# Bricktricker/gpu-solve

Measured on AMD Instinct MI355X. Metric: MLUPS (Jacobi smoother) + V-cycle wall-time, 512³ fp64; achieved HBM GB/s %peak, higher is better.
Workload: dtype f64

## Files before the change

### gpu-solve_amd/csrc/gs_capi.cpp

```cpp
#include <algorithm>
#include <array>
#include <chrono>
#include <cstdlib>
#include <cmath>
#include <cstring>
#include <iostream>
#include <memory>
#include <string>
#include <thread>
#include <vector>

#include <hip/hip_runtime.h>

#include "gpusolve_driver.h"
#include "gs_grid.hpp"

namespace {

thread_local std::string g_err;

template <class F>
int guarded(F&& f)
{
    try {
// ... 136 lines not shown
        if (residual) *residual = r;
    });
}

int gs_grid_jacobi(void* grid, int level, int sweeps)
{
    return guarded([&] { gs::HipSolver::jacobi(G(grid), (std::size_t)level, (std::size_t)sweeps); });
}

int gs_grid_residual_norm(void* grid, int level, double* norm)
{
    return guarded([&] {
        const double r = gs::HipSolver::compResidual(G(grid), (std::size_t)level, false, true);
        if (norm) *norm = r;
    });
}

int gs_grid_num_levels(void* grid) { return (int)G(grid).numLevels(); }

int gs_grid_level_fused(void* grid, int level)
{
    if (level < 0 || level >= (int)G(grid).numLevels()) return 0;
    return G(grid).getLevel(level).fusedPairs ? 1 : 0;
}

int gs_grid_level(void* grid, int level, gs_level* out)
{
    if (level < 0 || level >= (int)G(grid).numLevels() || !out) return 1;
    *out = G(grid).getLevel(level).geom;
    return 0;
}

static double* field_ptr(void* grid, int level, int field, bool writable)
{
    auto& g = G(grid);
    if (level < 0 || level >= (int)g.numLevels()) return nullptr;
    auto& L = g.getLevel(level);
    switch (field) {
    case 0: return L.v ? L.v.data() : nullptr;
    case 1: return L.restV ? L.restV.data() : nullptr;
    case 2:
        if (writable) g.newtonVTouched();
        return L.newtonV ? L.newtonV.data() : nullptr;
    case 3: return L.f ? L.f.data() : nullptr;
    case 4: return L.r ? L.r.data() : nullptr;
    case 5: return (level == 0 && g.newtonF) ? g.newtonF.data() : nullptr;
// ... 388 lines not shown
```

### gpu-solve_amd/csrc/gs_device.hpp

```cpp
#pragma once
#include <hip/hip_runtime.h>
#include <math.h>

#include <cmath>
#include <stdint.h>
#include <stdlib.h>

#include <map>
#include <mutex>
#include <utility>

#include "gpusolve_hip.h"

#ifdef GS_EXP_NOEXP
#define exp(x) ((x) * 1.0000001)
#endif
#ifdef GS_EXP_NOBAR
#define GS_LDS_BARRIER() __builtin_amdgcn_s_waitcnt(0xc07f)
#else
#define GS_LDS_BARRIER()                                                                                               \
    do {                                                                                                               \
        __builtin_amdgcn_s_waitcnt(0xc07f);                                                                            \
        __builtin_amdgcn_s_barrier();                                                                                  \
    } while (0)
// ... 118 lines not shown
{
    const unsigned e = ((unsigned)__double2hiint(s) >> 20) & 0x7ffu;
    if (k.fastdiv && e - 124u < 1500u) {
        const double y = hh_recip(k.hh);
        const double q = s * y;
        const double r = __builtin_fma(-k.hh, q, s);
        return __builtin_fma(r, y, q);
    }
    return s / k.hh;
}

__device__ __forceinline__ bool div_hh_fast_ok(double s)
{
    const unsigned e = ((unsigned)__double2hiint(s) >> 20) & 0x7ffu;
    return e - 124u < 1500u;
}
template <int N>
__device__ __forceinline__ void div_hh_n(const Coef& k, double (&s)[N])
{
    bool ok = k.fastdiv;
#pragma unroll
    for (int i = 0; i < N; i++) ok &= div_hh_fast_ok(s[i]);
    if (ok) {
        const double y = hh_recip(k.hh);
#pragma unroll
        for (int i = 0; i < N; i++) {
            const double q = s[i] * y;
            const double r = __builtin_fma(-k.hh, q, s[i]);
            s[i] = __builtin_fma(r, y, q);
        }
    } else {
#pragma unroll
        for (int i = 0; i < N; i++) s[i] = s[i] / k.hh;
    }
}

template <int MODE>
__device__ __forceinline__ void div_hh_row(const Coef& k, double (&q)[2])
{
    if (MODE == GS_NEWTON) {
        q[0] = div_hh(k, q[0]);
        q[1] = div_hh(k, q[1]);
    } else {
        div_hh_n(k, q);
    }
}
// ... 2329 lines not shown
        if (lane == 0) red[wid] = sumsq;
        __syncthreads();
        if (tid == 0) {
            double t = 0.0;
            for (int i = 0; i < 2 * WX; i++) t += red[i];
            partials[tile] = t;
        }
    }
    if constexpr (TS) {
        if (tid == 0) {
            double* t = const_cast<double*>(es) + 4 * tile;
            t[0] = (double)tstart;
            t[1] = (double)wall_clock64();
            t[2] = (double)(blockIdx.x + (int64_t)gridDim.x * blockIdx.y);
            t[3] = (double)(unsigned)__builtin_amdgcn_s_getreg((31 << 11) | 4);
        }
    }
}

constexpr int TBY_RY = 2, TBY_RY_NEWTON = 2, TBY_WX = 4, TB_RY_B = 2, TB_WX_B = 8;
constexpr int tby_pfd(int mode) { return mode == GS_LINEAR ? 2 : 1; }
bool tbx_pfd2() { return kKnobs.tbxPfd2; }

bool xh_enabled() { return kKnobs.pairXh; }

int64_t resident_blocks(const void* fn, int threads)
{
    static std::mutex m;
    static std::map<std::pair<const void*, int>, int64_t> cache;
    std::lock_guard<std::mutex> lk(m);
    const auto key = std::make_pair(fn, threads);
    auto it = cache.find(key);
    if (it != cache.end()) return it->second;
    int per = 0, dev = 0, cus = 0;
    if (hipOccupancyMaxActiveBlocksPerMultiprocessor(&per, fn, threads, 0) != hipSuccess || per < 1) per = 1;
    if (hipGetDevice(&dev) != hipSuccess ||
        hipDeviceGetAttribute(&cus, hipDeviceAttributeMultiprocessorCount, dev) != hipSuccess || cus < 1)
        cus = 256;
    (void)hipGetLastError();
    return cache[key] = (int64_t)per * cus;
}

int fit_chunk(int64_t tiles, int64_t planes, int64_t cap, int lo, int hi, bool even, double halo)
{
    if (!kKnobs.fitRounds || tiles < 1 || planes < 1 || cap < 1) return 0;
    double best = -1.0;
// ... 178 lines not shown
```

### gpu-solve_amd/csrc/gs_grid.cpp

```cpp
#include "gs_grid.hpp"

#include <algorithm>
#include <chrono>
#include <cmath>
#include <cstdio>
#include <cstdlib>
#include <iostream>
#include <string>
#include <utility>

#include <hip/hip_runtime.h>

#include "gpusolve_driver.h"

namespace gs {

void check(int code, const char* what)
{
    if (code != 0) throw Error(std::string(what) + ": " + gs_strerror(code));
}

DeviceField::DeviceField(int64_t nx, int64_t ny, int64_t nz, hipStream_t s, bool dry) : dry_(dry)
{
    int64_t origin = 0;
// ... 142 lines not shown
    const int nlev = (int)std::floor(std::log((double)mn) / std::log(2.0)) + 1;
    levels_.resize(nlev);
    for (int i = 0; i < 7; i++) {
        stencilAbi.s[i] = stencil.values[i];
        stencilAbi.ox[i] = stencil.getXOffset(i);
        stencilAbi.oy[i] = stencil.getYOffset(i);
        stencilAbi.oz[i] = stencil.getZOffset(i);
    }
    {
        auto on = [](const char* name) { return std::getenv(name) != nullptr; };
        sw.fusedSweeps = !on("GS_NO_FUSED_SWEEPS");
        sw.speculation = !on("GS_NO_SPECULATION");
        sw.fusedProlong = !on("GS_NO_FUSED_PROLONG");
        sw.fusedRR = !on("GS_NO_FUSED_RR");
        sw.zeroGuess = !on("GS_NO_ZERO_GUESS");
        sw.pipeline = !on("GS_NO_PIPELINE");
        sw.newtonFusedUpdate = !on("GS_NO_NEWTON_FUSED_UPDATE");
        sw.newtonB = !on("GS_NO_NEWTON_B");
        if (const char* e = std::getenv("GS_NEWTON_B_FUSED")) sw.newtonBFused = std::atoi(e) != 0;
        sw.newtonG = !on("GS_NO_NEWTON_G");
        if (const char* e = std::getenv("GS_NEWTON_PRO_POINTS")) sw.newtonProPoints = std::strtoll(e, nullptr, 10);
        if (const char* e = std::getenv("GS_TILE_POINTS")) sw.tilePoints = std::strtoll(e, nullptr, 10);
        if (const char* e = std::getenv("GS_HALO_ORDER")) sw.haloOrder = std::atoi(e);
    }
    std::vector<int64_t> nzs, pts;
    for (int l = 0; l < nlev; l++) {
        LevelData& L = levels_[l];
        L.levelDim = l == 0 ? gridDim
                            : std::array<std::size_t, 3>{levels_[l - 1].levelDim[0] / 2, levels_[l - 1].levelDim[1] / 2,
                                                         levels_[l - 1].levelDim[2] / 2};
        nzs.push_back((int64_t)L.levelDim[2]);
        pts.push_back((int64_t)(L.levelDim[0] * L.levelDim[1] * L.levelDim[2]));
    }
    if (agglomeratePoints < 0) {
        const char* e = std::getenv("GS_ZSLAB_MIN_POINTS");
        agglomeratePoints = e ? std::atoll(e) : 32768;
    }
    const SlabPlan plan = planZSlabs(nzs, pts, nranks(), agglomeratePoints);

    const hipStream_t s = stream_.s;
    int64_t maxParts = 1;
    for (int l = 0; l < nlev; l++) {
        LevelData& L = levels_[l];
        const int64_t nx = (int64_t)L.levelDim[0], ny = (int64_t)L.levelDim[1];
        L.distributed = plan.distributed[l];
        L.ranksLo = plan.lo[l];
// ... 5 lines not shown
            L.lo = 1;
            L.hi = (int64_t)L.levelDim[2];
        }
        const int64_t nz = L.hi - L.lo + 1;
        L.h = 1.0 / (L.levelDim[1] + 1);
        L.v = DeviceField(nx, ny, nz, s, dry);
        L.vAlt = DeviceField(nx, ny, nz, s, dry);
        L.f = DeviceField(nx, ny, nz, s, dry);
        if (l + 1 < nlev) L.r = DeviceField(nx, ny, nz, s, dry);
        if (mode == NONLINEAR && l > 0) L.restV = DeviceField(nx, ny, nz, s, dry);
        if (mode == NEWTON) L.newtonV = DeviceField(nx, ny, nz, s, dry);
        if (mode == NEWTON && sw.newtonB && dry) L.bfac = DeviceField(nx, ny, nz, s, dry);
        if (mode == NEWTON && l == 1 && nlev >= 3 && !L.distributed) L.newtonVNext = DeviceField(nx, ny, nz, s, dry);
        L.geom = gs_level{nx, ny, nz, L.v.ldy(), L.v.ldz(), L.lo - 1, L.h};
        maxParts = std::max(maxParts, gs_residual_num_partials(&stencilAbi, &L.geom));
        maxParts = std::max(maxParts, gs_jacobi_sweep2_num_partials(&stencilAbi, &L.geom, (int)mode));
        L.minPlanes = nz;
        if (L.distributed)
            for (int q = 0; q < nranks(); q++) L.minPlanes = std::min(L.minPlanes, L.ranksHi[q] - L.ranksLo[q] + 1);
        gs_level thin = L.geom;
        thin.nz = L.minPlanes;
        L.fusedPairs = sw.fusedSweeps && gs_jacobi_sweep2_supported_mode(&stencilAbi, &thin, (int)mode) == 2 &&
                       (!L.distributed || L.minPlanes >= 2);
        L.tiled = !L.distributed && pts[l] <= sw.tilePoints &&
                  gs_tiled_supported(&stencilAbi, &L.geom, (int)mode) != 0;
    }
    coarseFrom = levels_.size();
    {
        const char* e = std::getenv("GS_COARSE_POINTS");
        const int64_t thr = e ? std::atoll(e) : 512;
        if (thr > 0 && preSmoothing + postSmoothing < (1u << 20))
            for (int l = nlev - 1; l >= 1; l--) {
                if (levels_[l].distributed || pts[l] > thr || nlev - l > gs_coarse_cycle_max_levels()) break;
                coarseFrom = (std::size_t)l;
            }
    }
    if (mode == NEWTON) newtonF = DeviceField(levels_[0].geom.nx, levels_[0].geom.ny, levels_[0].geom.nz, s, dry);
    newtonVZero_ = mode == NEWTON;
    {
        const char* e = std::getenv("GS_METRICS");
        clock.on = !dry && e && *e && *e != '0';
        clock.levelMs.assign(nlev, 0.0);
    }
    if (dry) {
        dryParts_.assign(16, 0.0);
        partials_ = dryParts_.data();
// ... 213 lines not shown
int64_t pairPlanes(HipGridData& g, HipGridData::LevelData& L, int64_t z1, int64_t z2, hipStream_t s,
                   double* partials = nullptr)
{
    if (z2 < z1) return 0;
    gs_level sub = L.geom;
    sub.nz = z2 - z1 + 1;
    sub.z0 += z1 - 1;
    const int64_t off = (z1 - 1) * L.geom.ldz;
    const bool dist = L.distributed && g.nranks() > 1;
    const int zlo = z1 > 1 || (dist && g.rank() > 0);
    const int zhi = z2 < L.geom.nz || (dist && g.rank() + 1 < g.nranks());
    if (g.trace) {
        g.rec("pair", {{"L", (long long)g.levelIndex(L)}, {"z1", z1}, {"z2", z2}, {"zlo", zlo}, {"zhi", zhi},
                       {"vzero", L.vZero}, {"norm", partials != nullptr}});
        return partials ? 1 : 0;
    }
    check(gs_jacobi_sweep2_norm(&g.stencilAbi, &sub, g.kmode(), g.omega, g.gamma, L.vZero ? nullptr : L.v.data() + off,
                                L.vAlt.data() + off, L.f.data() + off, g.wOf(L) ? g.wOf(L) + off : nullptr,
                                zlo, zhi, partials, s),
          "gs_jacobi_sweep2");
    return partials ? gs_jacobi_sweep2_num_partials(&g.stencilAbi, &sub, (int)g.mode) : 0;
}

void proPlanes(HipGridData& g, HipGridData::LevelData& F, HipGridData::LevelData& C, int64_t z1, int64_t z2,
               hipStream_t s)
{
    if (z2 < z1) return;
    gs_level sub = F.geom;
    sub.nz = z2 - z1 + 1;
    sub.z0 += z1 - 1;
    const int64_t off = (z1 - 1) * F.geom.ldz;
    const bool dist = F.distributed && g.nranks() > 1;
    const int zlo = z1 > 1 || (dist && g.rank() > 0);
    const int zhi = z2 < F.geom.nz || (dist && g.rank() + 1 < g.nranks());
    if (g.trace) {
        g.rec("pro", {{"L", (long long)g.levelIndex(F)}, {"z1", z1}, {"z2", z2}, {"zlo", zlo}, {"zhi", zhi}});
        return;
    }
    const int64_t wsn = gs_jacobi_sweep2_prolong_ws_elems(&g.stencilAbi, &sub, (int)g.mode);
    DeviceBuf& wb = F.proWs[s == g.stream() ? 0 : 1];
    if (wsn > wb.size()) throw Error("gs_jacobi_sweep2_prolong: workspace not sized at grid creation");
    double* ws = wsn > 0 ? wb.get(wsn) : nullptr;
    check(gs_jacobi_sweep2_prolong_ws(&g.stencilAbi, &sub, g.kmode(), g.omega, g.gamma, F.v.data() + off,
                                      C.v.data(), nullptr, &C.geom, F.vAlt.data() + off, F.f.data() + off,
                                      g.wOf(F) ? g.wOf(F) + off : nullptr, zlo, zhi, ws, wsn, s),
          "gs_jacobi_sweep2_prolong");
// ... 167 lines not shown
        if ((F.ranksLo[q] - 1) % 2 != 0) return false;
        if (C.distributed && 2 * (C.ranksLo[q] - 1) != F.ranksLo[q] - 1) return false;
    }
    return !C.distributed || grid.vDepth(C) == 2;
}

static bool proWorthIt(HipGridData& grid, std::size_t l)
{
    if (grid.mode != GridParams::NEWTON) return true;
    const int64_t minPoints = grid.sw.newtonProPoints;
    const auto& F = grid.getLevel(l);
    return (int64_t)F.levelDim[0] * (int64_t)F.levelDim[1] * F.minPlanes >= minPoints;
}

void HipSolver::jacobi(HipGridData& grid, std::size_t l, std::size_t sweeps)
{
    auto& L = grid.getLevel(l);
    const hipStream_t s = grid.stream();
    const bool dist = L.distributed && grid.nranks() > 1;
    const int64_t nz = L.geom.nz;
    const int depth = grid.vDepth(L);
    int step = 0;
    while (sweeps > 0) {
        const bool pair = L.fusedPairs && sweeps >= 2;
        const int64_t b = pair ? 2 : depth;
        auto run = [&](int64_t z1, int64_t z2, hipStream_t st) {
            if (pair) pairPlanes(grid, L, z1, z2, st);
            else sweepPlanes(grid, L, z1, z2, st);
        };
        if (!dist) {
            run(1, nz, s);
        } else if (grid.overlapHalo && nz >= 2 * b + 1) {
            hipStream_t bs = s;
            const bool interiorFirst = step > 0 && !grid.haloReady();
            if (!grid.trace) {
                bs = grid.bndStream_.s;
                check((int)hipEventRecord(grid.evA_, s), "hipEventRecord");
            }
            auto interior = [&] {
                if (!grid.trace && step > 0)
                    check((int)hipStreamWaitEvent(s, grid.evBnd_[(step - 1) & 1], 0), "hipStreamWaitEvent");
                run(b + 1, nz - b, s);
            };
            if (interiorFirst) interior();
            if (step > 0) settleExchange(grid);
            if (!grid.trace) {
// ... 532 lines not shown
```

### gpu-solve_amd/csrc/gs_grid.hpp

```cpp
#pragma once
#include <array>
#include <cstddef>
#include <cstdint>
#include <initializer_list>
#include <memory>
#include <string>
#include <functional>
#include <vector>

#include "gpusolve_hip.h"
#include "gs_comm.hpp"
#include "gs_params.hpp"

namespace gs {

void check(int code, const char* what);

class DeviceField {
public:
    DeviceField() = default;
    DeviceField(int64_t nx, int64_t ny, int64_t nz, hipStream_t s, bool dry = false);
    ~DeviceField();
    DeviceField(const DeviceField&) = delete;
    DeviceField& operator=(const DeviceField&) = delete;
// ... 43 lines not shown
    std::vector<hipEvent_t> ev;
    std::vector<int> segLevel;
    void mark(hipStream_t s, int level, bool begin);
    void collect();
    ~LevelClock();
};

class HipGridData final : public GridParams {
public:
    struct LevelData {
        DeviceField v;
        DeviceField vAlt;
        DeviceField restV;
        DeviceField newtonV;
        DeviceField newtonVNext;
        DeviceField f;
        DeviceField r;
        DeviceField bfac;
        std::array<std::size_t, 3> levelDim{};
        double h = 0.0;
        gs_level geom{};
        bool distributed = false;
        bool fusedPairs = false;
        bool vZero = false;
        bool tiled = false;
        int64_t lo = 1, hi = 0;
        int64_t minPlanes = 0;
        std::vector<int64_t> ranksLo, ranksHi;
        std::unique_ptr<DeviceBuf[]> proWs = std::make_unique<DeviceBuf[]>(2);
    };

    explicit HipGridData(const GridParams& grid, Comm* comm = nullptr, int64_t agglomeratePoints = -1,
                         std::vector<std::string>* trace = nullptr);
    ~HipGridData();

    LevelData& getLevel(std::size_t l) { return levels_[l]; }
    const LevelData& getLevel(std::size_t l) const { return levels_[l]; }
    std::size_t numLevels() const { return levels_.size(); }

    DeviceField newtonF;
    gs_stencil stencilAbi{};
    hipStream_t stream() const { return stream_.s; }
    hipStream_t commStream() const { return commStream_.s; }
    Comm* comm() const { return comm_; }
    int rank() const { return comm_ ? comm_->rank() : 0; }
    int nranks() const { return comm_ ? comm_->size() : 1; }
    bool overlapHalo = true;
    struct Switches {
        bool fusedSweeps = true;
        bool speculation = true;
        bool fusedProlong = true;
        bool fusedRR = true;
        bool zeroGuess = true;
        bool pipeline = true;
        bool newtonFusedUpdate = true;
        bool newtonB = true;
        bool newtonBFused = true;
        bool newtonG = true;
        int64_t tilePoints = (int64_t)1 << 18;
        int64_t newtonProPoints = (int64_t)1 << 21;
        int haloOrder = 0;
    } sw;
    std::size_t coarseFrom = 0;
    LevelClock clock;
    std::vector<std::string>* trace = nullptr;
    void rec(const char* op, std::initializer_list<std::pair<const char*, long long>> kv, const char* field = nullptr);
    std::size_t levelIndex(const LevelData& L) const { return (std::size_t)(&L - levels_.data()); }
    static const char* fieldName(const LevelData& L, const DeviceField& f);

    double* partials() const { return partials_; }
    double* dNorm() const { return dNorm_; }
    double* hNormDev() const { return hNormDev_; }
    double* dRankSums() const { return dRankSums_; }
    double readNorm();
    void readNormBegin();
    double readNormEnd();
    void sync();

    int kmode() const { return newtonB_ ? (bconst_ ? (int)GS_NEWTON_G : (int)GS_NEWTON_B) : (int)mode; }
    const double* wOf(const LevelData& L) const
    {
        return newtonB_ ? L.bfac.data() : (L.newtonV ? L.newtonV.data() : nullptr);
    }
// ... 90 lines not shown
```

### gpu-solve_amd/csrc/gs_kernels.hip

```cpp
#include "gs_device.hpp"

extern "C" {

int gs_field_layout(int64_t nx, int64_t ny, int64_t nz, int64_t* ldy, int64_t* ldz, int64_t* alloc_elems,
                    int64_t* origin_offset)
{
    if (nx < 0 || ny < 0 || nz < 0 || !ldy || !ldz || !alloc_elems || !origin_offset) return GS_EINVAL;
    const int64_t py = ((nx + 2 + 15) / 16) * 16;
    *ldy = py;
    *ldz = py * (ny + 2);
    *origin_offset = 15 + *ldz;
    *alloc_elems = *ldz * (nz + 4) + 32;
    return 0;
}

int gs_rhs_init(const gs_level* L, double* f, int mode, double h0, double gamma, hipStream_t st)
{
    if (bad_level(L) || !f) return GS_EINVAL;
    const dim3 g((unsigned)((L->nx + 2 + 63) / 64), (unsigned)((L->ny + 2 + 3) / 4), (unsigned)(L->nz + 2)), b(64, 4);
    hipLaunchKernelGGL(k_rhs, g, b, 0, st, f, mode, h0, gamma, (int)L->nx, (int)L->ny, (int)L->nz, L->z0, L->ldy,
                       L->ldz);
    return launch_status();
}

// ... 121 lines not shown
            if (zv) GS_TBY(GS_LINEAR, true);
            else GS_TBY(GS_LINEAR, false);
        } else if (mode == GS_NONLINEAR) GS_TBY(GS_NONLINEAR, false);
        else if (mode == GS_NEWTON_B && zv) GS_TBY(GS_NEWTON_B, true);
        else if (mode == GS_NEWTON_B) GS_TBY(GS_NEWTON_B, false);
        else if (zv) GS_TBY(GS_NEWTON, true);
        else GS_TBY(GS_NEWTON, false);
    } else {
        if (mode == GS_LINEAR) {
            if (zv) GS_TB(GS_LINEAR, true);
            else GS_TB(GS_LINEAR, false);
        } else if (mode == GS_NONLINEAR) GS_TB(GS_NONLINEAR, false);
        else if (mode == GS_NEWTON_B && zv) GS_TB(GS_NEWTON_B, true);
        else if (mode == GS_NEWTON_B) GS_TB(GS_NEWTON_B, false);
        else if (zv) GS_TB(GS_NEWTON, true);
        else GS_TB(GS_NEWTON, false);
    }
#undef GS_TBX
#undef GS_TBX1
#undef GS_TBY
#undef GS_TBY1
#undef GS_TBY2
#undef GS_TB
    return launch_status();
}

int gs_jacobi_sweep2_prolong_supported(const gs_stencil* S, const gs_level* L, int mode)
{
    int zc;
    dim3 g, b;
    bool y2 = false, xh = false;
    mode = base_mode(mode);
    return !bad_level(L) && valid_stencil(S) && (mode == GS_LINEAR || newtonish(mode)) && L->z0 % 2 == 0 &&
           tb2_plan(S, L, &zc, &g, &b, &y2, mode, &xh, true) && (y2 || xh);
}

int64_t gs_jacobi_sweep2_prolong_ws_elems(const gs_stencil* S, const gs_level* L, int mode)
{
    int zc;
    dim3 g, b;
    bool y2 = false, xh = false;
    mode = base_mode(mode);
    if (!gs_jacobi_sweep2_prolong_supported(S, L, mode) || !tb2_plan(S, L, &zc, &g, &b, &y2, mode, &xh, true) || !xh)
        return 0;
    const int64_t bw = 2 * WAVE * TBY_WX, nb = (L->nx + bw - 1) / bw - 1;
    return nb * (L->nz + 4) * 4 * (L->ny + 2);
// ... 492 lines not shown
        L.ldz = g->ldz;
        L.nx = (int)g->nx;
        L.ny = (int)g->ny;
        L.nz = (int)g->nz;
        L.vz = a.v_zero != 0;
        L.k = make_coef(S, g, omega, gamma);
    }
    if (mode == GS_LINEAR) hipLaunchKernelGGL(k_coarse_cycle<GS_LINEAR>, dim3(1), dim3(CC_T), 0, st, P);
    else if (mode == GS_NONLINEAR) hipLaunchKernelGGL(k_coarse_cycle<GS_NONLINEAR>, dim3(1), dim3(CC_T), 0, st, P);
    else if (mode == GS_NEWTON_B) hipLaunchKernelGGL(k_coarse_cycle<GS_NEWTON_B>, dim3(1), dim3(CC_T), 0, st, P);
    else hipLaunchKernelGGL(k_coarse_cycle<GS_NEWTON>, dim3(1), dim3(CC_T), 0, st, P);
    return launch_status();
}

const char* gs_strerror(int code)
{
    if (code == 0) return "success";
    if (code == GS_EINVAL) return "gpusolve: invalid argument";
    return hipGetErrorString((hipError_t)code);
}

const char* gs_build_info(void)
{
    return "gpusolve_hip v13: pairs k_tb2y(4x2 waves, 2 rows/wave, one round of z-chunks on large levels, LINEAR 2-step prefetch; +prolong; "
           "512-point column blocks for longer rows in every mode; from 64^3 levels; zero-iterate chunks fitted to "
           "resident rounds; zero iterates q = +0; whole-wave rows without range selects (FX); LINEAR loads grouped by "
           "field; x-edge values in VGPRs for LINEAR and the NEWTON_B whole-row plain pair), sweeps k_rb(ry2 w4 zc<=32 "
           "dpp nt), fused residual+restriction (2 coarse rows per block from 2^26 points, descending z-chunks, halo rows "
           "loaded first, non-temporal unshared rows), NEWTON update + "
           "compF (+ level-1 restriction, + the next factor B), NEWTON inner solves on B (GS_NEWTON_B: reciprocal "
           "quotient, shared per pair; GS_NEWTON_G: B = gamma unread), unit-neighbour stencil sums, tiled small levels, "
           "one-workgroup coarse cycle; fp-contract=off";
}

}

#ifdef GS_EXP_EFIELD
extern "C" void gs_exp_set_efoff(int64_t n) { gs_exp_efoff = n; }
#endif
```

### gpu-solve_amd/gpusolve/_abi.py

```python
import ctypes as C
import os

PKG_ROOT = os.path.dirname(os.path.dirname(os.path.abspath(__file__)))
LIB_DIR = os.path.join(PKG_ROOT, "lib")
BIN_DIR = os.path.join(PKG_ROOT, "bin")
KERNEL_LIB = os.path.join(LIB_DIR, "libgpusolve_hip.so")
DIAG_LIB = os.path.join(LIB_DIR, "libgpusolve_diag.so")
DRIVER_LIB = os.path.join(LIB_DIR, "libgpusolve_driver.so")
EXECUTABLE = os.path.join(BIN_DIR, "GpuSolve-hip")

GS_LINEAR, GS_NONLINEAR, GS_NEWTON = 0, 1, 2
GS_NEWTON_B = 3
GS_NEWTON_G = 4
GS_EINVAL = 100001

dptr = C.POINTER(C.c_double)
i64 = C.c_int64


class gs_stencil(C.Structure):
    _fields_ = [("s", C.c_double * 7), ("ox", C.c_int * 7), ("oy", C.c_int * 7), ("oz", C.c_int * 7)]


class gs_level(C.Structure):
# ... 6 lines not shown


class gs_params(C.Structure):
    _fields_ = [("maxiter", i64), ("tol", C.c_double), ("dims", i64 * 3), ("mode", C.c_int), ("pre", i64),
                ("post", i64), ("omega", C.c_double), ("gamma", C.c_double), ("stencil", gs_stencil)]


KERNEL_API = {
    "gs_field_layout": (C.c_int, [i64, i64, i64, C.POINTER(i64), C.POINTER(i64), C.POINTER(i64), C.POINTER(i64)]),
    "gs_rhs_init": (C.c_int, [C.POINTER(gs_level), C.c_void_p, C.c_int, C.c_double, C.c_double, C.c_void_p]),
    "gs_jacobi_sweep": (C.c_int, [C.POINTER(gs_stencil), C.POINTER(gs_level), C.c_int, C.c_double, C.c_double,
                                  C.c_void_p, C.c_void_p, C.c_void_p, C.c_void_p, C.c_void_p]),
    "gs_jacobi_sweep_norm": (C.c_int, [C.POINTER(gs_stencil), C.POINTER(gs_level), C.c_int, C.c_double, C.c_double,
                                       C.c_void_p, C.c_void_p, C.c_void_p, C.c_void_p, C.c_void_p, C.c_void_p]),
    "gs_jacobi_sweep2_supported": (C.c_int, [C.POINTER(gs_stencil), C.POINTER(gs_level)]),
    "gs_jacobi_sweep2_supported_mode": (C.c_int, [C.POINTER(gs_stencil), C.POINTER(gs_level), C.c_int]),
    "gs_jacobi_sweep2": (C.c_int, [C.POINTER(gs_stencil), C.POINTER(gs_level), C.c_int, C.c_double, C.c_double,
                                   C.c_void_p, C.c_void_p, C.c_void_p, C.c_void_p, C.c_int, C.c_int, C.c_void_p]),
    "gs_jacobi_sweep2_norm": (C.c_int, [C.POINTER(gs_stencil), C.POINTER(gs_level), C.c_int, C.c_double,
                                        C.c_double, C.c_void_p, C.c_void_p, C.c_void_p, C.c_void_p, C.c_int,
                                        C.c_int, C.c_void_p, C.c_void_p]),
    "gs_jacobi_sweep2_num_partials": (i64, [C.POINTER(gs_stencil), C.POINTER(gs_level), C.c_int]),
    "gs_jacobi_sweep2_kernel": (C.c_char_p, [C.POINTER(gs_stencil), C.POINTER(gs_level), C.c_int]),
    "gs_jacobi_sweep2_prolong_supported": (C.c_int, [C.POINTER(gs_stencil), C.POINTER(gs_level), C.c_int]),
    "gs_jacobi_sweep2_prolong": (C.c_int, [C.POINTER(gs_stencil), C.POINTER(gs_level), C.c_int, C.c_double, C.c_double,
                                           C.c_void_p, C.c_void_p, C.c_void_p, C.POINTER(gs_level), C.c_void_p,
                                           C.c_void_p, C.c_void_p, C.c_int, C.c_int, C.c_void_p]),
    "gs_jacobi_sweep2_prolong_ws_elems": (i64, [C.POINTER(gs_stencil), C.POINTER(gs_level), C.c_int]),
    "gs_jacobi_sweep2_prolong_ws": (C.c_int, [C.POINTER(gs_stencil), C.POINTER(gs_level), C.c_int, C.c_double,
                                              C.c_double, C.c_void_p, C.c_void_p, C.c_void_p, C.POINTER(gs_level),
                                              C.c_void_p, C.c_void_p, C.c_void_p, C.c_int, C.c_int, C.c_void_p, i64,
                                              C.c_void_p]),
    "gs_residual": (C.c_int, [C.POINTER(gs_stencil), C.POINTER(gs_level), C.c_int, C.c_double, C.c_void_p,
                              C.c_void_p, C.c_void_p, C.c_void_p, C.c_void_p, C.c_void_p]),
    "gs_residual_num_partials": (i64, [C.POINTER(gs_stencil), C.POINTER(gs_level)]),
    "gs_sumsq_finish": (C.c_int, [C.c_void_p, i64, C.c_void_p, C.c_int, C.c_void_p]),
    "gs_restrict": (C.c_int, [C.c_void_p, C.POINTER(gs_level), C.c_void_p, C.POINTER(gs_level), C.c_void_p]),
    "gs_residual_restrict": (C.c_int, [C.POINTER(gs_stencil), C.POINTER(gs_level), C.c_int, C.c_double,
                                       C.c_void_p, C.c_void_p, C.c_void_p, C.c_void_p, C.c_void_p,
                                       C.POINTER(gs_level), C.c_void_p]),
    "gs_residual_restrict_slab_supported": (C.c_int, [C.POINTER(gs_stencil), C.POINTER(gs_level)]),
    "gs_residual_restrict_slab": (C.c_int, [C.POINTER(gs_stencil), C.POINTER(gs_level), C.c_int, C.c_double,
                                            C.c_void_p, C.c_void_p, C.c_void_p, C.c_void_p, C.c_void_p,
                                            C.POINTER(gs_level), C.c_int, C.c_void_p]),
    "gs_tiled_supported": (C.c_int, [C.POINTER(gs_stencil), C.POINTER(gs_level), C.c_int]),
    "gs_smooth2_restrict_tiled": (C.c_int, [C.POINTER(gs_stencil), C.POINTER(gs_level), C.c_int, C.c_double,
# ... 24 lines not shown
    "gs_newton_bfac": (C.c_int, [C.POINTER(gs_level), C.c_double, C.c_void_p, C.c_void_p, C.c_void_p]),
    "gs_newton_F_update": (C.c_int, [C.POINTER(gs_stencil), C.POINTER(gs_level), C.c_double, C.c_void_p, C.c_void_p,
                                     C.c_void_p, C.c_void_p, C.c_void_p, C.c_void_p, C.c_void_p]),
    "gs_fill": (C.c_int, [C.c_void_p, C.c_double, i64, C.c_void_p]),
    "gs_copy": (C.c_int, [C.c_void_p, C.c_void_p, i64, C.c_void_p]),
    "gs_axpy": (C.c_int, [C.c_void_p, C.c_void_p, C.c_double, i64, C.c_void_p]),
    "gs_coarse_cycle_max_levels": (C.c_int, []),
    "gs_coarse_cycle": (C.c_int, [C.POINTER(gs_stencil), C.POINTER(gs_coarse_level), C.c_int, C.c_int, C.c_double,
                                  C.c_double, C.c_int, C.c_int, C.c_void_p]),
    "gs_strerror": (C.c_char_p, [C.c_int]),
    "gs_build_info": (C.c_char_p, []),
}

DRIVER_API = {
    "gs_parse_config": (C.c_int, [C.c_char_p, C.POINTER(gs_params)]),
    "gs_grid_create": (C.c_void_p, [C.POINTER(gs_params)]),
    "gs_grid_destroy": (None, [C.c_void_p]),
    "gs_grid_solve": (C.c_int, [C.c_void_p, C.c_int, dptr, C.c_int, C.POINTER(C.c_int)]),
    "gs_grid_vcycle": (C.c_int, [C.c_void_p, dptr]),
    "gs_grid_jacobi": (C.c_int, [C.c_void_p, C.c_int, C.c_int]),
    "gs_grid_residual_norm": (C.c_int, [C.c_void_p, C.c_int, dptr]),
    "gs_grid_num_levels": (C.c_int, [C.c_void_p]),
    "gs_grid_level_fused": (C.c_int, [C.c_void_p, C.c_int]),
    "gs_grid_level": (C.c_int, [C.c_void_p, C.c_int, C.POINTER(gs_level)]),
    "gs_grid_field": (C.c_void_p, [C.c_void_p, C.c_int, C.c_int]),
    "gs_grid_stream": (C.c_void_p, [C.c_void_p]),
    "gs_grid_download": (C.c_int, [C.c_void_p, C.c_int, C.c_int, dptr]),
    "gs_grid_upload": (C.c_int, [C.c_void_p, C.c_int, C.c_int, dptr]),
    "gs_grid_sync": (C.c_int, [C.c_void_p]),
    "gs_grid_comm_stats": (C.c_int, [C.c_void_p, dptr, C.POINTER(C.c_int64)]),
    "gs_grid_comm_stats_max": (C.c_int, [C.c_void_p, dptr]),
    "gs_grid_metrics": (C.c_int, [C.c_void_p, C.c_char_p, C.c_int, dptr, C.c_int]),
    "gs_dump_write": (C.c_int, [dptr, i64, i64, i64, C.c_char_p]),
    "gs_grid_dump": (C.c_int, [C.c_void_p, C.c_int, C.c_int, C.c_char_p]),
    "gs_grid_time_jacobi": (C.c_int, [C.c_void_p, C.c_int, C.c_int, C.c_int, C.POINTER(C.c_float)]),
    "gs_grid_time_vcycles": (C.c_int, [C.c_void_p, C.c_int, dptr, dptr]),
    "gs_zslab_plan": (C.c_int, [C.POINTER(i64), C.c_int, i64, C.c_int, C.POINTER(C.c_int), C.POINTER(i64),
                                C.POINTER(i64)]),
    "gs_zslab_schedule": (C.c_int, [C.POINTER(gs_params), C.c_int, C.c_int, i64, C.c_char_p, i64, C.POINTER(i64)]),
    "gs_rccl_unique_id": (C.c_int, [C.POINTER(C.c_ubyte)]),
    "gs_uid_publish": (C.c_int, [C.c_char_p, C.POINTER(C.c_ubyte)]),
    "gs_uid_default_path": (C.c_int, [C.c_char_p, C.c_int]),
    "gs_uid_await": (C.c_int, [C.c_char_p, C.c_double, C.POINTER(C.c_ubyte)]),
    "gs_grid_create_rccl": (C.c_void_p, [C.POINTER(gs_params), C.c_int, C.c_int, C.POINTER(C.c_ubyte)]),
    "gs_grid_create_rccl_ctas": (C.c_void_p, [C.POINTER(gs_params), C.c_int, C.c_int, C.POINTER(C.c_ubyte), C.c_int]),
    "gs_grid_comm_ctas": (C.c_int, [C.c_void_p]),
# ... 74 lines not shown
```

### include/gpusolve_driver.h

```cpp
#ifndef GPUSOLVE_DRIVER_H
#define GPUSOLVE_DRIVER_H

#include <stdint.h>
#include "gpusolve_hip.h"

#ifdef __cplusplus
extern "C" {
#endif

typedef struct {
    int64_t maxiter;
    double tol;
    int64_t dims[3];
    int mode;
    int64_t pre, post;
    double omega, gamma;
    gs_stencil stencil;
} gs_params;

int gs_parse_config(const char* text, gs_params* out);

void* gs_grid_create(const gs_params* p);
void gs_grid_destroy(void* grid);

int gs_grid_solve(void* grid, int print, double* hist, int cap, int* count);

int gs_grid_vcycle(void* grid, double* residual);
int gs_grid_jacobi(void* grid, int level, int sweeps);
int gs_grid_residual_norm(void* grid, int level, double* norm);
int gs_grid_num_levels(void* grid);
int gs_grid_level_fused(void* grid, int level);
int gs_grid_level(void* grid, int level, gs_level* out);
double* gs_grid_field(void* grid, int level, int field);
hipStream_t gs_grid_stream(void* grid);
int gs_grid_download(void* grid, int level, int field, double* host);
int gs_grid_upload(void* grid, int level, int field, const double* host);
int gs_grid_sync(void* grid);
int gs_grid_comm_stats(void* grid, double* halo_host_ms, int64_t* halo_calls);
int gs_grid_comm_stats_max(void* grid, double* halo_host_max_ms);
int gs_grid_metrics(void* grid, char* line, int cap, double* level_ms, int levels_cap);
int gs_dump_write(const double* host, int64_t px, int64_t py, int64_t pz, const char* path);
int gs_grid_dump(void* grid, int level, int field, const char* path);

int gs_grid_time_jacobi(void* grid, int level, int warmup, int sweeps, float* ms);
int gs_grid_time_vcycles(void* grid, int cycles, double* ms, double* last_residual);

int gs_zslab_plan(const int64_t dims[3], int nranks, int64_t min_points, int max_levels, int* distributed,
                  int64_t* lo, int64_t* hi);
int gs_zslab_schedule(const gs_params* p, int nranks, int rank, int64_t min_points, char* buf, int64_t cap,
                      int64_t* len);
int gs_rccl_unique_id(unsigned char uid[128]);
void* gs_grid_create_rccl(const gs_params* p, int rank, int nranks, const unsigned char uid[128]);
void* gs_grid_create_rccl_ctas(const gs_params* p, int rank, int nranks, const unsigned char uid[128], int ctas);
int gs_grid_comm_ctas(void* grid);
// ... 17 lines not shown
```

### include/gpusolve_hip.h

```cpp
#ifndef GPUSOLVE_HIP_H
#define GPUSOLVE_HIP_H

#include <stdint.h>
#include <hip/hip_runtime_api.h>

#ifdef __cplusplus
extern "C" {
#endif

#define GS_EINVAL 100001

enum { GS_LINEAR = 0, GS_NONLINEAR = 1, GS_NEWTON = 2 };
enum { GS_NEWTON_B = 3 };
enum { GS_NEWTON_G = 4 };

typedef struct {
    double s[7];
    int ox[7], oy[7], oz[7];
} gs_stencil;

typedef struct {
    int64_t nx, ny, nz;
    int64_t ldy, ldz;
    int64_t z0;
// ... 1 lines not shown
} gs_level;

int gs_field_layout(int64_t nx, int64_t ny, int64_t nz, int64_t* ldy, int64_t* ldz, int64_t* alloc_elems,
                    int64_t* origin_offset);

int gs_rhs_init(const gs_level* L, double* f, int mode, double h0, double gamma, hipStream_t stream);

int gs_jacobi_sweep(const gs_stencil* S, const gs_level* L, int mode, double omega, double gamma,
                    const double* v_in, double* v_out, const double* f, const double* w, hipStream_t stream);

int gs_jacobi_sweep_norm(const gs_stencil* S, const gs_level* L, int mode, double omega, double gamma,
                         const double* v_in, double* v_out, const double* f, const double* w, double* partials,
                         hipStream_t stream);

int gs_jacobi_sweep2_supported(const gs_stencil* S, const gs_level* L);
int gs_jacobi_sweep2_supported_mode(const gs_stencil* S, const gs_level* L, int mode);
int gs_jacobi_sweep2(const gs_stencil* S, const gs_level* L, int mode, double omega, double gamma,
                     const double* v_in, double* v_out, const double* f, const double* w, int zlo, int zhi,
                     hipStream_t stream);
int gs_jacobi_sweep2_norm(const gs_stencil* S, const gs_level* L, int mode, double omega, double gamma,
                          const double* v_in, double* v_out, const double* f, const double* w, int zlo, int zhi,
                          double* partials, hipStream_t stream);
int64_t gs_jacobi_sweep2_num_partials(const gs_stencil* S, const gs_level* L, int mode);
int gs_jacobi_sweep2_prolong_supported(const gs_stencil* S, const gs_level* L, int mode);
int gs_jacobi_sweep2_prolong(const gs_stencil* S, const gs_level* L, int mode, double omega, double gamma,
                             const double* v_in, const double* coarse_v, const double* coarse_sub,
                             const gs_level* coarse, double* v_out, const double* f, const double* w, int zlo,
                             int zhi, hipStream_t stream);
int64_t gs_jacobi_sweep2_prolong_ws_elems(const gs_stencil* S, const gs_level* L, int mode);
int gs_jacobi_sweep2_prolong_ws(const gs_stencil* S, const gs_level* L, int mode, double omega, double gamma,
                                const double* v_in, const double* coarse_v, const double* coarse_sub,
                                const gs_level* coarse, double* v_out, const double* f, const double* w, int zlo,
                                int zhi, double* ws, int64_t ws_elems, hipStream_t stream);
int gs_tiled_supported(const gs_stencil* S, const gs_level* L, int mode);
int gs_smooth2_restrict_tiled(const gs_stencil* S, const gs_level* fine, int mode, double omega, double gamma,
                              const double* v_in, double* v_out, const double* f, const double* w, double* coarse_f,
                              const gs_level* coarse, hipStream_t stream);
int gs_prolong_smooth2_tiled(const gs_stencil* S, const gs_level* fine, int mode, double omega, double gamma,
                             const double* v_in, const double* coarse_v, const gs_level* coarse, double* v_out,
                             const double* f, const double* w, hipStream_t stream);
const char* gs_jacobi_sweep2_kernel(const gs_stencil* S, const gs_level* L, int mode);

int gs_residual(const gs_stencil* S, const gs_level* L, int mode, double gamma, const double* v, const double* f,
                const double* w, double* r, double* partials, hipStream_t stream);
int64_t gs_residual_num_partials(const gs_stencil* S, const gs_level* L);

// ... 66 lines not shown
```

Baseline: 482,700.

## Add three-sweep temporally blocked Jacobi kernel for large linear levels

Adds a k_tb3y kernel that performs three Jacobi sweeps per pass over a z-streamed tile, keeping intermediate sweep rows, previous-plane values and f rows in registers and LDS, so v and f are read from HBM once for every three sweeps. The level driver uses it on large, non-distributed LINEAR levels when three or at least five sweeps remain. It also adds a min/max exponent check that decides the fast-division path per batch. The cost is more LDS and register pressure, barriers per plane, and redundant halo computation, which may lower occupancy.

```diff
diff --git a/gpu-solve_amd/csrc/gs_capi.cpp b/gpu-solve_amd/csrc/gs_capi.cpp
--- a/gpu-solve_amd/csrc/gs_capi.cpp
+++ b/gpu-solve_amd/csrc/gs_capi.cpp
@@ -182,6 +182,12 @@
 {
     if (level < 0 || level >= (int)G(grid).numLevels()) return 0;
     return G(grid).getLevel(level).fusedPairs ? 1 : 0;
+}
+
+int64_t gs_grid_level_triples(void* grid, int level)
+{
+    if (level < 0 || level >= (int)G(grid).numLevels()) return 0;
+    return G(grid).getLevel(level).triplesRun;
 }
 
 int gs_grid_level(void* grid, int level, gs_level* out)
diff --git a/gpu-solve_amd/csrc/gs_device.hpp b/gpu-solve_amd/csrc/gs_device.hpp
--- a/gpu-solve_amd/csrc/gs_device.hpp
+++ b/gpu-solve_amd/csrc/gs_device.hpp
@@ -164,6 +164,30 @@
 #pragma unroll
     for (int i = 0; i < N; i++) ok &= div_hh_fast_ok(s[i]);
     if (ok) {
+        const double y = hh_recip(k.hh);
+#pragma unroll
+        for (int i = 0; i < N; i++) {
+            const double q = s[i] * y;
+            const double r = __builtin_fma(-k.hh, q, s[i]);
+            s[i] = __builtin_fma(r, y, q);
+        }
+    } else {
+#pragma unroll
+        for (int i = 0; i < N; i++) s[i] = s[i] / k.hh;
+    }
+}
+
+template <int N>
+__device__ __forceinline__ void div_hh_mm(const Coef& k, double (&s)[N])
+{
+    unsigned lo = 0x7ffu, hi = 0u;
+#pragma unroll
+    for (int i = 0; i < N; i++) {
+        const unsigned e = ((unsigned)__double2hiint(s[i]) >> 20) & 0x7ffu;
+        lo = min(lo, e);
+        hi = max(hi, e);
+    }
+    if (k.fastdiv && lo >= 124u && hi <= 1623u) {
         const double y = hh_recip(k.hh);
 #pragma unroll
         for (int i = 0; i < N; i++) {
@@ -2539,6 +2563,223 @@
 constexpr int tby_pfd(int mode) { return mode == GS_LINEAR ? 2 : 1; }
 bool tbx_pfd2() { return kKnobs.tbxPfd2; }
 
+template <bool UN, bool FX, bool DB>
+__global__ __launch_bounds__(WAVE* TBY_WX * 2) void k_tb3y(Coef k, const double* __restrict__ v,
+                                                           const double* __restrict__ f, double* __restrict__ out,
+                                                           int nx, int ny, int nz, int64_t ldy, int64_t ldz, int ZC)
+{
+    constexpr int MODE = GS_LINEAR, RY = TBY_RY, WXMAX = TBY_WX;
+    static_assert(RY == 2, "k_tb3y: two rows per y-wave (the boundary tests below name the rows)");
+    constexpr int N0 = RY + 2;
+    constexpr int N1 = RY + 1;
+    constexpr int NE = N0 + N1 + RY;
+    constexpr int B1 = DB ? 2 : 1, B2 = DB ? N1 : 1, B3 = DB ? RY : 1;
+    __shared__ double edge[2][2][WXMAX + 2][2][NE];
+    __shared__ double2 yrow[2][2][WXMAX][3][WAVE];
+    __shared__ double2 f1_l[N1][2 * WXMAX][WAVE];
+    __shared__ double2 f2_l[RY][2 * WXMAX][WAVE];
+    __shared__ double2 s1p_l[N1][2 * WXMAX][WAVE];
+    __shared__ double2 s2p_l[RY][2 * WXMAX][WAVE];
+    const int lane = threadIdx.x;
+    const int wy = __builtin_amdgcn_readfirstlane(threadIdx.z);
+    const int WX = blockDim.y;
+    const int wx = __builtin_amdgcn_readfirstlane(threadIdx.y);
+    const int wid = wx + WXMAX * wy;
+    const int tid = threadIdx.x + WAVE * (threadIdx.y + WX * threadIdx.z);
+    for (int i = tid; i < 2 * 2 * (WXMAX + 2) * 2 * NE; i += WAVE * WX * 2) (&edge[0][0][0][0][0])[i] = 0.0;
+    __syncthreads();
+    const int64_t tile = xcd_tile(blockIdx.x + (int64_t)gridDim.x * blockIdx.y, (int64_t)gridDim.x * gridDim.y);
+    const int x = 1 + wx * (2 * WAVE) + 2 * lane;
+    const int xl = min(x, nx + 1);
+    const bool bx0 = !FX && x > nx, bx1 = !FX && x + 1 > nx;
+    const bool okx0 = FX || x <= nx, okx1 = FX || x + 1 <= nx;
+    const int y0 = 1 + (int)(tile % gridDim.x) * (2 * RY);
+    const int zb = 1 + (int)(tile / gridDim.x) * ZC;
+    const int ze = min(zb + ZC - 1, nz);
+    const bool mir = wy != 0;
+    auto yof = [&](int j) { return mir ? y0 + 2 * RY - j : y0 - 1 + j; };
+
+    int64_t roff[RY + 3];
+    bool rowc[RY + 3];
+#pragma unroll
+    for (int j = -2; j <= RY; j++) {
+        const int y = yof(j);
+        roff[j + 2] = (int64_t)min(max(y, 0), ny + 1) * ldy;
+        rowc[j + 2] = y >= 1 && y <= ny;
+    }
+    const bool in1 = rowc[1] && rowc[2] && rowc[3] && rowc[4];
+    const bool in2 = rowc[2] && rowc[3] && rowc[4];
+    auto planeok = [&](int z) { return z >= 1 && z <= nz; };
+    auto cz = [&](int z) { return min(max(z, 0), nz + 1); };
+    auto at = [&](const double* base, int j, int z) { return base + xl + roff[j + 2] + (int64_t)z * ldz; };
+
+    double2 Vp[N0], Vc[N0], VL[2][N0], FL[2][N0], HL[2];
+    double2 S1c[N0], S2c[N1];
+#pragma unroll
+    for (int i = 0; i < N0; i++) S1c[i] = make_double2(0.0, 0.0);
+#pragma unroll
+    for (int i = 0; i < N1; i++) {
+        S2c[i] = make_double2(0.0, 0.0);
+        f1_l[i][wid][lane] = make_double2(0.0, 0.0);
+        s1p_l[i][wid][lane] = make_double2(0.0, 0.0);
+    }
+#pragma unroll
+    for (int i = 0; i < RY; i++) {
+        f2_l[i][wid][lane] = make_double2(0.0, 0.0);
+        s2p_l[i][wid][lane] = make_double2(0.0, 0.0);
+    }
+    auto load_slot = [&](const int s, const int z, const int zv) {
+        HL[s] = ld2(at(v, -2, z));
+#pragma unroll
+        for (int i = 0; i < N0; i++) VL[s][i] = ld2(at(v, i - 1, zv));
+#pragma unroll
+        for (int i = 0; i < N0; i++) FL[s][i] = ld2(at(f, i - 1, z));
+    };
+#pragma unroll
+    for (int i = 0; i < N0; i++) {
+        Vp[i] = ld2(at(v, i - 1, cz(zb - 3)));
+        Vc[i] = ld2(at(v, i - 1, cz(zb - 2)));
+    }
+    load_slot(1, cz(zb - 2), cz(zb - 1));
+    for (int z0 = zb - 2; z0 <= ze + 2; z0 += 2) {
+#pragma unroll
+        for (int ph = 0; ph < 2; ph++) {
+            const int z = z0 + ph;
+            const int cs = ph ^ 1;
+            load_slot(ph, cz(z + 1), cz(z + 2));
+            if (lane == 0) {
+#pragma unroll
+                for (int i = 0; i < N0; i++) edge[ph][wy][wx + 1][0][i] = Vc[i].x;
+#pragma unroll
+                for (int i = 0; i < N1; i++) edge[ph][wy][wx + 1][0][N0 + i] = S1c[i + 1].x;
+#pragma unroll
+                for (int i = 0; i < RY; i++) edge[ph][wy][wx + 1][0][N0 + N1 + i] = S2c[i + 1].x;
+            }
+            if (lane == WAVE - 1) {
+#pragma unroll
+                for (int i = 0; i < N0; i++) edge[ph][wy][wx + 1][1][i] = Vc[i].y;
+#pragma unroll
+                for (int i = 0; i < N1; i++) edge[ph][wy][wx + 1][1][N0 + i] = S1c[i + 1].y;
+#pragma unroll
+                for (int i = 0; i < RY; i++) edge[ph][wy][wx + 1][1][N0 + N1 + i] = S2c[i + 1].y;
+            }
+            yrow[ph][wy][wx][0][lane] = Vc[N0 - 1];
+            yrow[ph][wy][wx][1][lane] = S1c[N0 - 1];
+            yrow[ph][wy][wx][2][lane] = S2c[N1 - 1];
+            GS_LDS_BARRIER();
+            double CL[NE], CR[NE];
+#pragma unroll
+            for (int i = 0; i < NE; i++) {
+                CL[i] = uniform_d(edge[ph][wy][wx][1][i]);
+                CR[i] = uniform_d(edge[ph][wy][wx + 2][0][i]);
+            }
+            const double2 vY = yrow[ph][wy ^ 1][wx][0][lane];
+            const double2 s1Y = yrow[ph][wy ^ 1][wx][1][lane];
+            const double2 s2Y = yrow[ph][wy ^ 1][wx][2][lane];
+
+            auto row_sums = [&](auto mirc, const double2 c, const double2 lm, const double2 lp, const double2 zm,
+                                const double2 zp, const double el, const double er, double& q0, double& q1) {
+                constexpr bool M = decltype(mirc)::get();
+                const double2 ym = M ? lp : lm, yp = M ? lm : lp;
+                const double xm0 = lane_from_left<true>(c.y, el);
+                const double xp1 = lane_from_right<true>(c.x, er);
+                q0 = stencil_sum<UN>(k, c.x, c.y, xm0, yp.x, ym.x, zp.x, zm.x);
+                q1 = stencil_sum<UN>(k, c.y, xp1, c.x, yp.y, ym.y, zp.y, zm.y);
+            };
+            auto row_finish = [&](const double2 c, const double q0, const double q1, const double2 fv) {
+                const double a0 = op_finish<MODE>(k, q0, c.x, 0.0);
+                const double a1 = op_finish<MODE>(k, q1, c.y, 0.0);
+                return make_double2(jacobi_update<MODE>(k, c.x, fv.x - a0, 0.0),
+                                    jacobi_update<MODE>(k, c.y, fv.y - a1, 0.0));
+            };
+            auto kept = [&](const bool keep, const double2 c, const double2 n) {
+                return make_double2((keep || bx0) ? c.x : n.x, (keep || bx1) ? c.y : n.y);
+            };
+            double2 S1n[N0], S2n[N1], F1[N1];
+            const bool pz0 = planeok(z), pz1 = planeok(z - 1);
+            auto sweeps = [&](auto mirc) {
+                static_assert(N0 % B1 == 0 && N1 % B2 == 0 && RY % B3 == 0, "whole division batches");
+#pragma unroll
+                for (int b = 0; b < N0; b += B1) {
+                    double q[2 * B1];
+#pragma unroll
+                    for (int i = b; i < b + B1; i++)
+                        row_sums(mirc, Vc[i], i == 0 ? HL[cs] : Vc[i - 1], i == N0 - 1 ? vY : Vc[i + 1], Vp[i], VL[cs][i],
+                                 CL[i], CR[i], q[2 * (i - b)], q[2 * (i - b) + 1]);
+                    div_hh_mm(k, q);
+#pragma unroll
+                    for (int i = b; i < b + B1; i++) S1n[i] = row_finish(Vc[i], q[2 * (i - b)], q[2 * (i - b) + 1], FL[cs][i]);
+                }
+                if (!FX || !pz0 || !in1) {
+#pragma unroll
+                    for (int i = 0; i < N0; i++) S1n[i] = kept(!pz0 || !rowc[i + 1], Vc[i], S1n[i]);
+                }
+#pragma unroll
+                for (int b = 0; b < N1; b += B2) {
+                    double q[2 * B2];
+#pragma unroll
+                    for (int i = b; i < b + B2; i++) {
+                        F1[i] = f1_l[i][wid][lane];
+                        row_sums(mirc, S1c[i + 1], S1c[i], i == N1 - 1 ? s1Y : S1c[i + 2], s1p_l[i][wid][lane], S1n[i + 1],
+                                 CL[N0 + i], CR[N0 + i], q[2 * (i - b)], q[2 * (i - b) + 1]);
+                    }
+                    div_hh_mm(k, q);
+#pragma unroll
+                    for (int i = b; i < b + B2; i++)
+                        S2n[i] = row_finish(S1c[i + 1], q[2 * (i - b)], q[2 * (i - b) + 1], F1[i]);
+                }
+                if (!FX || !pz1 || !in2) {
+#pragma unroll
+                    for (int i = 0; i < N1; i++) S2n[i] = kept(!pz1 || !rowc[i + 2], S1c[i + 1], S2n[i]);
+                }
+                if (z - 2 >= zb && z - 2 <= ze) {
+                    const int64_t zo = (int64_t)(z - 2) * ldz;
+#pragma unroll
+                    for (int b = 1; b <= RY; b += B3) {
+                        double q[2 * B3];
+                        double2 fv[B3];
+#pragma unroll
+                        for (int j = b; j < b + B3; j++) {
+                            fv[j - b] = f2_l[j - 1][wid][lane];
+                            row_sums(mirc, S2c[j], S2c[j - 1], j == RY ? s2Y : S2c[j + 1], s2p_l[j - 1][wid][lane], S2n[j],
+                                     CL[N0 + N1 + j - 1], CR[N0 + N1 + j - 1], q[2 * (j - b)], q[2 * (j - b) + 1]);
+                        }
+                        div_hh_mm(k, q);
+#pragma unroll
+                        for (int j = b; j < b + B3; j++) {
+                            const double2 o = row_finish(S2c[j], q[2 * (j - b)], q[2 * (j - b) + 1], fv[j - b]);
+                            if (yof(j) <= ny) {
+                                double* qo = out + x + roff[j + 2] + zo;
+                                if (okx1) st2s<true>(qo, o.x, o.y);
+                                else if (okx0) *qo = o.x;
+                            }
+                        }
+                    }
+                }
+            };
+            if (mir) sweeps(BoolC<true>{});
+            else sweeps(BoolC<false>{});
+#pragma unroll
+            for (int j = 1; j <= RY; j++) {
+                s2p_l[j - 1][wid][lane] = S2c[j];
+                f2_l[j - 1][wid][lane] = F1[j];
+            }
+#pragma unroll
+            for (int i = 0; i < N1; i++) {
+                S2c[i] = S2n[i];
+                s1p_l[i][wid][lane] = S1c[i + 1];
+                f1_l[i][wid][lane] = FL[cs][i + 1];
+            }
+#pragma unroll
+            for (int i = 0; i < N0; i++) {
+                S1c[i] = S1n[i];
+                Vp[i] = Vc[i];
+                Vc[i] = VL[cs][i];
+            }
+        }
+    }
+}
+
 bool xh_enabled() { return kKnobs.pairXh; }
 
 int64_t resident_blocks(const void* fn, int threads)
diff --git a/gpu-solve_amd/csrc/gs_grid.cpp b/gpu-solve_amd/csrc/gs_grid.cpp
--- a/gpu-solve_amd/csrc/gs_grid.cpp
+++ b/gpu-solve_amd/csrc/gs_grid.cpp
@@ -188,6 +188,8 @@
         if (const char* e = std::getenv("GS_NEWTON_PRO_POINTS")) sw.newtonProPoints = std::strtoll(e, nullptr, 10);
         if (const char* e = std::getenv("GS_TILE_POINTS")) sw.tilePoints = std::strtoll(e, nullptr, 10);
         if (const char* e = std::getenv("GS_HALO_ORDER")) sw.haloOrder = std::atoi(e);
+        sw.sweep3 = !on("GS_NO_SWEEP3");
+        if (const char* e = std::getenv("GS_SWEEP3_MIN_POINTS")) sw.sweep3MinPoints = std::strtoll(e, nullptr, 10);
     }
     std::vector<int64_t> nzs, pts;
     for (int l = 0; l < nlev; l++) {
@@ -239,6 +241,8 @@
         thin.nz = L.minPlanes;
         L.fusedPairs = sw.fusedSweeps && gs_jacobi_sweep2_supported_mode(&stencilAbi, &thin, (int)mode) == 2 &&
                        (!L.distributed || L.minPlanes >= 2);
+        L.fusedTriples = sw.sweep3 && sw.fusedSweeps && mode == LINEAR && !L.distributed && pts[l] >= sw.sweep3MinPoints &&
+                         gs_jacobi_sweep3_supported(&stencilAbi, &L.geom) == 2;
         L.tiled = !L.distributed && pts[l] <= sw.tilePoints &&
                   gs_tiled_supported(&stencilAbi, &L.geom, (int)mode) != 0;
     }
@@ -498,6 +502,12 @@
     return partials ? gs_jacobi_sweep2_num_partials(&g.stencilAbi, &sub, (int)g.mode) : 0;
 }
 
+void tripleLevel(HipGridData& g, HipGridData::LevelData& L, hipStream_t s)
+{
+    check(gs_jacobi_sweep3(&g.stencilAbi, &L.geom, g.omega, g.gamma, L.v.data(), L.vAlt.data(), L.f.data(), s),
+          "gs_jacobi_sweep3");
+}
+
 void proPlanes(HipGridData& g, HipGridData::LevelData& F, HipGridData::LevelData& C, int64_t z1, int64_t z2,
                hipStream_t s)
 {
@@ -711,6 +721,13 @@
     const int depth = grid.vDepth(L);
     int step = 0;
     while (sweeps > 0) {
+        if (L.fusedTriples && !dist && !grid.trace && !L.vZero && (sweeps == 3 || sweeps >= 5)) {
+            tripleLevel(grid, L, s);
+            L.triplesRun++;
+            L.v.swap(L.vAlt);
+            sweeps -= 3;
+            continue;
+        }
         const bool pair = L.fusedPairs && sweeps >= 2;
         const int64_t b = pair ? 2 : depth;
         auto run = [&](int64_t z1, int64_t z2, hipStream_t st) {
diff --git a/gpu-solve_amd/csrc/gs_grid.hpp b/gpu-solve_amd/csrc/gs_grid.hpp
--- a/gpu-solve_amd/csrc/gs_grid.hpp
+++ b/gpu-solve_amd/csrc/gs_grid.hpp
@@ -89,6 +89,8 @@
         gs_level geom{};
         bool distributed = false;
         bool fusedPairs = false;
+        bool fusedTriples = false;
+        int64_t triplesRun = 0;
         bool vZero = false;
         bool tiled = false;
         int64_t lo = 1, hi = 0;
@@ -126,6 +128,8 @@
         bool newtonG = true;
         int64_t tilePoints = (int64_t)1 << 18;
         int64_t newtonProPoints = (int64_t)1 << 21;
+        bool sweep3 = true;
+        int64_t sweep3MinPoints = (int64_t)1 << 26;
         int haloOrder = 0;
     } sw;
     std::size_t coarseFrom = 0;
diff --git a/gpu-solve_amd/csrc/gs_kernels.hip b/gpu-solve_amd/csrc/gs_kernels.hip
--- a/gpu-solve_amd/csrc/gs_kernels.hip
+++ b/gpu-solve_amd/csrc/gs_kernels.hip
@@ -167,6 +167,35 @@
 #undef GS_TBY1
 #undef GS_TBY2
 #undef GS_TB
+    return launch_status();
+}
+
+int gs_jacobi_sweep3_supported(const gs_stencil* S, const gs_level* L)
+{
+    int zc;
+    dim3 g, b;
+    bool y2 = false, xh = false;
+    if (!S || bad_level(L) || !valid_stencil(S) || L->z0 != 0) return 0;
+    const int q = tb2_plan(S, L, &zc, &g, &b, &y2, GS_LINEAR, &xh);
+    return y2 ? q : 0;
+}
+
+int gs_jacobi_sweep3(const gs_stencil* S, const gs_level* L, double omega, double gamma, const double* v_in,
+                     double* v_out, const double* f, hipStream_t st)
+{
+    int zc;
+    dim3 g, b;
+    bool y2 = false, xh = false;
+    if (!S || bad_level(L) || !valid_stencil(S) || L->z0 != 0 || !v_in || !v_out || !f || v_in == v_out ||
+        !tb2_plan(S, L, &zc, &g, &b, &y2, GS_LINEAR, &xh) || !y2)
+        return GS_EINVAL;
+    const Coef k = make_coef(S, L, omega, gamma);
+    const int nx = (int)L->nx, ny = (int)L->ny, nz = (int)L->nz;
+#define GS_TB3(U, X) hipLaunchKernelGGL((k_tb3y<U, X, U>), g, b, 0, st, k, v_in, f, v_out, nx, ny, nz, L->ldy, L->ldz, zc)
+    if (k.unit && kKnobs.pairFx && nx % (2 * WAVE) == 0) GS_TB3(true, true);
+    else if (k.unit) GS_TB3(true, false);
+    else GS_TB3(false, false);
+#undef GS_TB3
     return launch_status();
 }
 
@@ -705,7 +734,8 @@
 
 const char* gs_build_info(void)
 {
-    return "gpusolve_hip v13: pairs k_tb2y(4x2 waves, 2 rows/wave, one round of z-chunks on large levels, LINEAR 2-step prefetch; +prolong; "
+    return "gpusolve_hip v14: LINEAR triples k_tb3y(the pair's whole-row tile, three sweeps per pass, one-step prefetch, "
+           "per-lane f / previous-plane rows in LDS), pairs k_tb2y(4x2 waves, 2 rows/wave, one round of z-chunks on large levels, LINEAR 2-step prefetch; +prolong; "
            "512-point column blocks for longer rows in every mode; from 64^3 levels; zero-iterate chunks fitted to "
            "resident rounds; zero iterates q = +0; whole-wave rows without range selects (FX); LINEAR loads grouped by "
            "field; x-edge values in VGPRs for LINEAR and the NEWTON_B whole-row plain pair), sweeps k_rb(ry2 w4 zc<=32 "
diff --git a/gpu-solve_amd/gpusolve/_abi.py b/gpu-solve_amd/gpusolve/_abi.py
--- a/gpu-solve_amd/gpusolve/_abi.py
+++ b/gpu-solve_amd/gpusolve/_abi.py
@@ -52,6 +52,9 @@
                                         C.c_int, C.c_void_p, C.c_void_p]),
     "gs_jacobi_sweep2_num_partials": (i64, [C.POINTER(gs_stencil), C.POINTER(gs_level), C.c_int]),
     "gs_jacobi_sweep2_kernel": (C.c_char_p, [C.POINTER(gs_stencil), C.POINTER(gs_level), C.c_int]),
+    "gs_jacobi_sweep3_supported": (C.c_int, [C.POINTER(gs_stencil), C.POINTER(gs_level)]),
+    "gs_jacobi_sweep3": (C.c_int, [C.POINTER(gs_stencil), C.POINTER(gs_level), C.c_double, C.c_double,
+                                   C.c_void_p, C.c_void_p, C.c_void_p, C.c_void_p]),
     "gs_jacobi_sweep2_prolong_supported": (C.c_int, [C.POINTER(gs_stencil), C.POINTER(gs_level), C.c_int]),
     "gs_jacobi_sweep2_prolong": (C.c_int, [C.POINTER(gs_stencil), C.POINTER(gs_level), C.c_int, C.c_double, C.c_double,
                                            C.c_void_p, C.c_void_p, C.c_void_p, C.POINTER(gs_level), C.c_void_p,
@@ -122,6 +125,7 @@
     "gs_grid_residual_norm": (C.c_int, [C.c_void_p, C.c_int, dptr]),
     "gs_grid_num_levels": (C.c_int, [C.c_void_p]),
     "gs_grid_level_fused": (C.c_int, [C.c_void_p, C.c_int]),
+    "gs_grid_level_triples": (i64, [C.c_void_p, C.c_int]),
     "gs_grid_level": (C.c_int, [C.c_void_p, C.c_int, C.POINTER(gs_level)]),
     "gs_grid_field": (C.c_void_p, [C.c_void_p, C.c_int, C.c_int]),
     "gs_grid_stream": (C.c_void_p, [C.c_void_p]),
diff --git a/include/gpusolve_driver.h b/include/gpusolve_driver.h
--- a/include/gpusolve_driver.h
+++ b/include/gpusolve_driver.h
@@ -30,6 +30,7 @@
 int gs_grid_residual_norm(void* grid, int level, double* norm);
 int gs_grid_num_levels(void* grid);
 int gs_grid_level_fused(void* grid, int level);
+int64_t gs_grid_level_triples(void* grid, int level);
 int gs_grid_level(void* grid, int level, gs_level* out);
 double* gs_grid_field(void* grid, int level, int field);
 hipStream_t gs_grid_stream(void* grid);
diff --git a/include/gpusolve_hip.h b/include/gpusolve_hip.h
--- a/include/gpusolve_hip.h
+++ b/include/gpusolve_hip.h
@@ -47,6 +47,9 @@
                           const double* v_in, double* v_out, const double* f, const double* w, int zlo, int zhi,
                           double* partials, hipStream_t stream);
 int64_t gs_jacobi_sweep2_num_partials(const gs_stencil* S, const gs_level* L, int mode);
+int gs_jacobi_sweep3_supported(const gs_stencil* S, const gs_level* L);
+int gs_jacobi_sweep3(const gs_stencil* S, const gs_level* L, double omega, double gamma, const double* v_in,
+                     double* v_out, const double* f, hipStream_t stream);
 int gs_jacobi_sweep2_prolong_supported(const gs_stencil* S, const gs_level* L, int mode);
 int gs_jacobi_sweep2_prolong(const gs_stencil* S, const gs_level* L, int mode, double omega, double gamma,
                              const double* v_in, const double* coarse_v, const double* coarse_sub,
```

Result: faster. 493,200, median of 6 (+2.2%).
